# mdolab/adflow

Measured on AMD Instinct MI355X. Metric: Mcells*residual-evals/s, higher is better.
Workload: dtype f64

## Files before the change

adflow_amd/csrc/api.hip:

```cpp
#include <hip/hip_runtime.h>

#include <algorithm>
#include <cmath>
#include <cstdarg>
#include <cstdio>
#include <cstring>
#include <functional>
#include <array>
#include <map>
#include <string>
#include <tuple>
#include <vector>

#include "internal.h"
#include "flow_plan.h"

extern int g_march_kch, g_viscous_tiled, g_inviscid_march, g_roe_march, g_sa_march;
int g_test_fault = 0;
int g_rvec_joint = 1;
int g_pc_fused = 1;
int g_xcd_tiles = 2;

namespace {

// ... 2043 lines not shown
    if (!g_gf_nofit) {
        double tbest = 1.e300;
        const long Tmax = std::max<long>(N, planes / kmin);
        for (long m = 1; m * W <= Tmax + W; ++m) {
            std::vector<int> c;
            split(m * W, c);
            const double t = makespan(c);
            if (t < tbest - 1.e-9) { tbest = t; best = c; }
            if (m > 64) break;
        }
        std::vector<int> one(N, 1);
        if (makespan(one) < tbest) best = one;
    } else {
        best.resize(N);
        const int L = g_march_kch > 0 ? g_march_kch : 32;
        for (int q = 0; q < N; ++q) best[q] = (cols[q].nz + L - 1) / L;
    }
    struct Chunk { int col, k0, k1; };
    std::vector<Chunk> ch;
    for (int q = 0; q < N; ++q) {
        int k = 2;
        for (int e = 0; e < best[q]; ++e) {
            const int len = (cols[q].nz + best[q] - 1 - e) / best[q];
            if (len <= 0) continue;
            ch.push_back(Chunk{q, k, k + len - 1});
            k += len;
        }
    }
    std::stable_sort(ch.begin(), ch.end(), [&](const Chunk& a, const Chunk& b) {
        const int la = a.k1 - a.k0, lb = b.k1 - b.k0;
        if (la != lb) return la > lb;
        if (cols[a.col].slot != cols[b.col].slot) return cols[a.col].slot < cols[b.col].slot;
        if (a.k0 != b.k0) return a.k0 < b.k0;
        return a.col < b.col;
    });
    auto make_table = [&](const std::vector<Chunk>& list, std::pair<int4*, int>* out) -> int {
        const int T = (int)list.size();
        std::vector<int> ord;
        if (round_order(T, W, &ord)) return 1;
        std::vector<int4> phys(ord.size());
        for (size_t p = 0; p < ord.size(); ++p) {
            const int e = ord[p];
            int4 tt;
            if (e >= 0) {
                const Col& c = cols[list[e].col];
                tt.x = c.slot; tt.y = c.bx | (c.by << 16); tt.z = list[e].k0; tt.w = list[e].k1;
            } else { tt.x = -1; tt.y = tt.z = tt.w = 0; }
            phys[p] = tt;
        }
        int n = (int)phys.size();
        while (n > 0 && phys[n - 1].x < 0) --n;
        int4* d = nullptr;
        HIPCHK(hipMalloc((void**)&d, sizeof(int4) * std::max(n, 1)));
        if (n > 0) HIPCHK(hipMemcpy(d, phys.data(), sizeof(int4) * n, hipMemcpyHostToDevice));
        *out = std::make_pair(d, n);
        return 0;
    };
    if (make_table(ch, all)) return 1;
    std::vector<Chunk> in, bd;
    for (const Chunk& c : ch) {
        const Col& q = cols[c.col];
        const int il = q.nx + 1, jl = q.ny + 1, kl = q.nz + 1;
        const int ia = 2 + 60 * q.bx, ib_ = std::min(ia + 59, il), ja = 2 + R * q.by, jb_ = std::min(ja + R - 1, jl);
        const bool interior = (ia - reach >= 2 && ib_ + reach <= il && ja - reach >= 2 && jb_ + reach <= jl && c.k0 - reach >= 2 &&
                               c.k1 + reach <= kl);
        (interior ? in : bd).push_back(c);
    }
    if (make_table(in, in_) || make_table(bd, bd_)) return 1;
    return 0;
}

int ensure_gf_tiles(int level)
{
    if (g_gf_tiles.count(level)) return 0;
    std::pair<int4*, int> a, i, b;
    if (build_chunk_tables(level, 3, 1.5, 1, &a, &i, &b, 2)) return 1;
    g_gf_tiles[level] = a; g_gf_tiles_int[level] = i; g_gf_tiles_bnd[level] = b;
    return 0;
}

int ensure_sa_tiles(int level)
{
    if (g_sa_tiles.count(level)) return 0;
    std::pair<int4*, int> a, i, b;
    if (build_chunk_tables(level, 4, 0.5, 2, &a, &i, &b)) return 1;
    g_sa_tiles[level] = a; g_sa_tiles_int[level] = i; g_sa_tiles_bnd[level] = b;
    return 0;
}

int make_list_host(int level, const int32_t* blk, const int32_t* idx, int ld, int first, int n, std::vector<int>& hb,
                   std::vector<long>& ho)
{
    hb.resize(n);
    ho.resize(n);
    for (int t = 0; t < n; ++t) {
        const int nn = blk[first + t];
        Block* b = find_block(nn, level, 1);
        if (!b) return fail("comm pattern of level %d references unregistered block %d", level, nn);
        const int i = idx[first + t], j = idx[ld + first + t], k = idx[2 * ld + first + t];
        if (i < 0 || i > b->v.ib || j < 0 || j > b->v.jb || k < 0 || k > b->v.kb)
            return fail("comm pattern of level %d: cell (%d,%d,%d) outside block %d", level, i, j, k, nn);
        hb[t] = nn;
        ho[t] = b->v.idx(i, j, k);
    }
    return 0;
}

int upload_list(const std::vector<int>& hb, const std::vector<long>& ho, int** d_blk, long** d_off)
{
    const size_t n = hb.size();
    *d_blk = nullptr;
    *d_off = nullptr;
    if (n == 0) return 0;
    HIPCHK(hipMalloc((void**)d_blk, sizeof(int) * n));
    HIPCHK(hipMalloc((void**)d_off, sizeof(long) * n));
    HIPCHK(hipMemcpy(*d_blk, hb.data(), sizeof(int) * n, hipMemcpyHostToDevice));
    HIPCHK(hipMemcpy(*d_off, ho.data(), sizeof(long) * n, hipMemcpyHostToDevice));
    return 0;
}

int make_list(int level, const int32_t* blk, const int32_t* idx, int ld, int first, int n, int** d_blk, long** d_off)
{
    std::vector<int> hb;
    std::vector<long> ho;
    if (make_list_host(level, blk, idx, ld, first, n, hb, ho)) return 1;
    return upload_list(hb, ho, d_blk, d_off);
}

int build_comm(int level, int nLayers, CommPattern** out)
{
    auto it = g_comm.find(std::make_pair(level, nLayers));
    if (it == g_comm.end()) return fail("no %d-layer comm pattern registered for level %d", nLayers, level);
    CommPattern& cp = it->second;
    *out = &cp;
    if (ensure_table(level)) return 1;
    if (cp.built) return 0;
    const int nc = (int)cp.h_donorBlock.size();
    cp.local.n = nc;
    {
        std::vector<int> db, hb;
        std::vector<long> dof, hof;
        if (make_list_host(level, cp.h_donorBlock.data(), cp.h_donorIdx.data(), nc, 0, nc, db, dof)) return 1;
        if (make_list_host(level, cp.h_haloBlock.data(), cp.h_haloIdx.data(), nc, 0, nc, hb, hof)) return 1;
        std::vector<int> perm(nc);
        for (int t = 0; t < nc; ++t) perm[t] = t;
        std::sort(perm.begin(), perm.end(), [&](int a, int c) { return hb[a] != hb[c] ? hb[a] < hb[c] : hof[a] < hof[c]; });
        std::vector<int> db2(nc), hb2(nc);
        std::vector<long> dof2(nc), hof2(nc);
        for (int t = 0; t < nc; ++t) { db2[t] = db[perm[t]]; dof2[t] = dof[perm[t]]; hb2[t] = hb[perm[t]]; hof2[t] = hof[perm[t]]; }
        if (g_comm_self && nc > 0) {
            cp.local.n = 0;
            CommList s, r;
            s.n = r.n = nc;
            s.peer = r.peer = g_self_rank;
            if (upload_list(db2, dof2, &s.blkA, &s.offA)) return 1;
            if (upload_list(hb2, hof2, &r.blkA, &r.offA)) return 1;
            HIPCHK(hipMalloc((void**)&s.buf, sizeof(double) * 11 * (size_t)nc));
            HIPCHK(hipMalloc((void**)&r.buf, sizeof(double) * 11 * (size_t)nc));
            cp.sends.push_back(s);
            cp.recvs.push_back(r);
        } else {
            if (upload_list(db2, dof2, &cp.local.blkA, &cp.local.offA)) return 1;
            if (upload_list(hb2, hof2, &cp.local.blkB, &cp.local.offB)) return 1;
        }
    }
    const int ns = (int)cp.h_sendProc.size(), nr = (int)cp.h_recvProc.size();
// ... 3167 lines not shown
    if (need_ready()) return 1;
    if (!sums || n < 1 || n > 6) return fail("res_norms: n must be 1..6");
    if (!g_norm_dev) HIPCHK(hipMalloc((void**)&g_norm_dev, sizeof(double) * 8));
    HIPCHK(hipMemsetAsync(g_norm_dev, 0, sizeof(double) * 8, g_stream));
    int rc = for_level(level, [&](Block* b) {
        if (n > b->v.nw) return fail("res_norms: n=%d exceeds nw=%d", n, b->v.nw);
        launch_res_norms(b->v, n, g_norm_dev, g_stream);
        return 0;
    });
    if (rc) return rc;
#ifndef ADFLOW_NO_RCCL
    if (g_nccl && g_nranks > 1) NCCLCHK(ncclAllReduce(g_norm_dev, g_norm_dev, n, ncclDouble, ncclSum, g_nccl, g_stream));
#endif
    HIPCHK(hipMemcpyAsync(sums, g_norm_dev, sizeof(double) * n, hipMemcpyDeviceToHost, g_stream));
    HIPCHK(hipStreamSynchronize(g_stream));
    return 0;
}

int adflow_gpu_event_record(int slot)
{
    if (g_device < 0) return fail("adflow_gpu_init has not been called");
    if (slot < 0 || slot >= 64) return fail("event slot %d out of range", slot);
    HIPCHK(hipEventRecord(g_events[slot], g_stream));
    return 0;
}

int adflow_gpu_event_elapsed_ms(int a, int b, double* ms)
{
    if (a < 0 || a >= 64 || b < 0 || b >= 64 || !ms) return fail("bad event arguments");
    HIPCHK(hipEventSynchronize(g_events[b]));
    float f = 0.f;
    HIPCHK(hipEventElapsedTime(&f, g_events[a], g_events[b]));
    *ms = f;
    return 0;
}

int adflow_gpu_march_stats(int level, double* out, int n)
{
    if (need_ready()) return 1;
    if (!out || n < 4) return fail("march_stats: n = %d (>= 4)", n);
    for (int q = 0; q < n; ++q) out[q] = 0.0;
    if (ensure_gf_tiles(level) || ensure_sa_tiles(level) || ensure_tiles(level)) return 1;
    {
        const auto& tt = g_sa_tiles[level];
        std::vector<int4> h((size_t)tt.second);
        if (tt.second > 0) HIPCHK(hipMemcpy(h.data(), tt.first, sizeof(int4) * h.size(), hipMemcpyDeviceToHost));
        for (const int4& t : h)
            if (t.x >= 0) out[0] += 4.0 * (t.w - t.z + 1);
    }
    {
        const auto& tt = g_gf_tiles[level];
        std::vector<int4> h((size_t)tt.second);
        if (tt.second > 0) HIPCHK(hipMemcpy(h.data(), tt.first, sizeof(int4) * h.size(), hipMemcpyDeviceToHost));
        for (const int4& t : h)
            if (t.x >= 0) out[1] += 4.0 * (t.w - t.z + 3);
    }
    for (auto& kv : g_blocks) {
        if (std::get<0>(kv.first) != level || std::get<1>(kv.first) != 1) continue;
        const BlkView& v = kv.second->v;
        int ntx, nty, ntz;
        euler_march_tiles(v, &ntx, &nty, &ntz);
        out[2] += 4.0 * ntx * nty * (v.nz + ntz);
    }
    return 0;
}

int adflow_gpu_sync(void)
{
    if (g_device < 0) return fail("adflow_gpu_init has not been called");
    HIPCHK(hipGetLastError());
    HIPCHK(hipStreamSynchronize(g_stream));
    return 0;
}

int adflow_gpu_set_tuning(const char* key, int value)
{
    ++g_state_gen;
    if (!key) return fail("null tuning key");
    if (!strcmp(key, "euler_march")) { g_use_march = (value != 0); return 0; }
    if (!strcmp(key, "viscous_tiled")) { g_viscous_tiled = value; return 0; }
    if (!strcmp(key, "inviscid_march")) { g_inviscid_march = value; return 0; }
    if (!strcmp(key, "roe_march")) { g_roe_march = value; return 0; }
    if (!strcmp(key, "sa_march")) { g_sa_march = value; return 0; }
    if (!strcmp(key, "overlap")) { g_overlap = value; return 0; }
    if (!strcmp(key, "max_grid_z")) { g_max_grid_z = (value > 0) ? value : 65535; return 0; }
    if (!strcmp(key, "metric_from_x")) { g_metric_from_x = value; return 0; }
    if (!strcmp(key, "xcd_tiles")) {
        g_xcd_tiles = value;
        if (g_stream) (void)hipStreamSynchronize(g_stream);
        mg_graph_drop();
        for (auto& kv : g_tiles) (void)hipFree(kv.second.first);
        g_tiles.clear();
        return 0;
    }
    if (!strcmp(key, "phase_events")) {
        if (value != 0 && (value < 8 || value > 56)) return fail("phase_events: first slot must be 8..56 (or 0 = off)");
        g_phase_base = value;
        return 0;
    }
    if (!strcmp(key, "march_kch")) {
        if (value < 4) return fail("march_kch must be >= 4");
        g_march_kch = value;
        if (g_stream) (void)hipStreamSynchronize(g_stream);
        mg_graph_drop();
        for (auto* mp : {&g_tiles, &g_gf_tiles, &g_gf_tiles_int, &g_gf_tiles_bnd, &g_sa_tiles, &g_sa_tiles_int, &g_sa_tiles_bnd}) {
            for (auto& kv : *mp) (void)hipFree(kv.second.first);
            mp->clear();
        }
        return 0;
    }
    if (!strcmp(key, "split_eval")) { g_split_eval = value; return 0; }
    if (!strcmp(key, "test_fault")) { g_test_fault = value; g_mgg.failed = false; mg_graph_drop(); return 0; }
    if (!strcmp(key, "ad_cache")) { g_ad_cache = value; if (!value) { if (g_stream) (void)hipStreamSynchronize(g_stream); ad_drop(); } return 0; }
    if (!strcmp(key, "rvec_joint")) { g_rvec_joint = value; return 0; }
    if (!strcmp(key, "jac_snap")) { g_jac_snap = value; return 0; }
    if (!strcmp(key, "pc_fused")) { g_pc_fused = value; mg_graph_drop(); return 0; }
    if (!strcmp(key, "mg_graph")) { g_mg_graph = value; g_mgg.failed = false; mg_graph_drop(); return 0; }
    if (!strcmp(key, "comm_self")) {
        if (g_stream) (void)hipStreamSynchronize(g_stream);
        g_comm_self = value;
        for (auto& kv : g_comm) drop_comm_lists(kv.second);
        return 0;
    }
    if (!strcmp(key, "dadi_pcr")) { g_dadi_pcr = value; mg_graph_drop(); return 0; }
    if (!strcmp(key, "ra_pcr")) { g_ra_pcr = value; mg_graph_drop(); return 0; }
    if (!strcmp(key, "dadi_upd")) { g_dadi_upd = value; mg_graph_drop(); return 0; }
    if (!strcmp(key, "gf_cus")) {
        g_gf_nofit = (value < 0);
        g_num_cus = value > 0 ? value : 0;
        if (g_stream) (void)hipStreamSynchronize(g_stream);
        mg_graph_drop();
        for (auto* mp : {&g_tiles, &g_gf_tiles, &g_gf_tiles_int, &g_gf_tiles_bnd, &g_sa_tiles, &g_sa_tiles_int, &g_sa_tiles_bnd}) {
            for (auto& kv : *mp) (void)hipFree(kv.second.first);
            mp->clear();
        }
        return 0;
    }
    return fail("unknown tuning key '%s'", key);
}

int adflow_gpu_set_async(int on)
{
    g_async = (on != 0);
    return 0;
}

int adflow_gpu_abi_sizes(int* opts_bytes, int* desc_bytes)
{
    if (opts_bytes) *opts_bytes = (int)sizeof(adflow_opts);
    if (desc_bytes) *desc_bytes = (int)sizeof(adflow_block_desc);
    return 0;
}

int adflow_gpu_abi_sizes2(int* bc_subface_bytes, int* comm_pattern_bytes)
{
    if (bc_subface_bytes) *bc_subface_bytes = (int)sizeof(adflow_bc_subface);
    if (comm_pattern_bytes) *comm_pattern_bytes = (int)sizeof(adflow_comm_pattern);
    return 0;
}

}

static void free_side_buffers(void)
{
    free_xsurf();
    if (g_vec_dev) (void)hipFree(g_vec_dev);
    g_vec_dev = nullptr;
    g_vec_elems = 0;
    if (g_norm_dev) (void)hipFree(g_norm_dev);
    g_norm_dev = nullptr;
    if (g_floor_flag_dev) (void)hipFree(g_floor_flag_dev);
    g_floor_flag_dev = nullptr;
    if (g_snapreq.dev) (void)hipFree(g_snapreq.dev);
    g_snapreq = SnapReq();
#ifndef ADFLOW_NO_RCCL
    if (g_nccl) (void)ncclCommDestroy(g_nccl);
    g_nccl = nullptr;
    g_rank = 0;
    g_nranks = 1;
#endif
}
```

adflow_amd/csrc/internal.h:

```cpp
#pragma once
#include <hip/hip_runtime.h>
#include <stdint.h>
#include "../../include/adflow_gpu.h"

#define ADF_PAD0 14

#ifdef HOSTSIM
#define GPTR(T) T*
#else
#define GPTR(T) T __attribute__((address_space(1)))*
#endif

__device__ __forceinline__ double ldg(GPTR(const double) base, unsigned byteoff)
{
    return *(GPTR(const double))((GPTR(const char))base + byteoff);
}
__device__ __forceinline__ void stg(GPTR(double) base, unsigned byteoff, double v)
{
    *(GPTR(double))((GPTR(char))base + byteoff) = v;
}

#ifndef ADF_NR
#define ADF_NR 1
#endif
// ... 311 lines not shown

#include <vector>
struct PcTab {
    long ncell;
    double* fac;
    double* ws;
    const int* nbr;
    const int* vec;
    const int* cblk;
    const int* cbox;
    const JmBlk* blk;
    int* flag;
    int sten[7];
    const double* tsm;
    double turbDiag;
    int asmEnt[23];
    signed char tgt[121];
    double* wsx;
};
int launch_pc_factor(const PcTab& T, int nState, const std::vector<int>& planeStart, hipStream_t s);
enum { PC_MAXW = 4 };
int launch_pc_apply(const PcTab& T, int nState, int transpose, const std::vector<int>& planeStart, const double* r, double* z,
                    hipStream_t s, int nv = 1, long ldr = 0, long ldz = 0);
int launch_pcf_factor(const PcTab& T, int nState, int nEnt, const std::vector<int>& levelStart, hipStream_t s);
int launch_pcf_apply(const PcTab& T, int nState, int nEnt, int transpose, const std::vector<int>& levelStart, const double* r,
                     double* z, hipStream_t s, int nv = 1, long ldr = 0, long ldz = 0);
struct PcMgSten { int s[7]; };
void launch_mg_fine_copy(const JmBlk* src, const JmBlk* dst, int nslots, int maxnx, int maxny, int maxnz, int nState, const PcMgSten& S,
                         const double* tsm, double turbDiag, long N, hipStream_t s);
void launch_mg_coarsen(const JmBlk* fine, const JmBlk* coarse, int nslots, int maxnx, int maxny, int maxnz, int nState, const PcMgSten& S,
                       hipStream_t s);
void launch_mg_restrict(const JmBlk* fine, const JmBlk* coarse, int nslots, int maxnx, int maxny, int maxnz, int nState, const double* r,
                        double* rhs, hipStream_t s);
void launch_mg_residual(const JmBlk* tab, const JmBlk* coarse, int nslots, int maxnx, int maxny, int maxnz, int nState, int transpose,
                        const PcMgSten& S, const double* r, const double* x, double* y, double* res, hipStream_t s);
enum { GM_PARTS = 256 };
int gm_groups(long n);
void launch_gm_mgs(double* w, const double* v, const double* hp, const double* u, double* out, double* hOut, long n, hipStream_t s);
void launch_gm_sum(const double* hp, long n, double* hOut, hipStream_t s);
void launch_gm_axpby(double* y, double a, const double* x, double b, long n, hipStream_t s);
enum { GM_MAXV = 32 };
struct GmCoef { double a[GM_MAXV], b[GM_MAXV]; };
void launch_gm_mgs_multi(double* w, const double* v, const double* hp, const double* u, double* out, double* hOut, long n, long ld,
                         int nvec, hipStream_t s);
void launch_gm_sum_multi(const double* hp, long n, double* hOut, int nvec, hipStream_t s);
void launch_gm_axpby_multi(double* y, long ldy, const double* x, long ldx, const GmCoef& k, long n, int nvec, hipStream_t s);
struct KParams;
enum { ANK_PARTS = 256 };
enum AnkScal {
    ANK_H = 0, ANK_HINV = 1,
    ANK_SUMS = 2,
    ANK_LAMBDA = 5,
    ANK_NORM = 6,
    ANK_NSCAL = 8
};
enum AnkRed {
    ANK_RED_SUMS = 0,
    ANK_RED_MIN = 3 * ANK_PARTS,
    ANK_RED_SCAL = 4 * ANK_PARTS,
    ANK_RED = ANK_RED_SCAL + ANK_NSCAL
};
int ank_groups(long n);
void launch_ank_set_w(const BlkView* tab, int nslots, int maxnx, int maxny, int maxnz, int nS, const double* vec, const double* hv,
                      const double* hdev, const KParams* kp, int* floored, hipStream_t s);
void launch_ank_get_r(const BlkView* tab, int nslots, int maxnx, int maxny, int maxnz, int nS, double* vec, double turbScale, hipStream_t s);
void launch_ank_time_step(const BlkView* tab, int nslots, int maxnx, int maxny, int maxnz, double cfl, double* tsm, long N, hipStream_t s);
void launch_ank_quotient(const BlkView* tab, int nslots, int maxnx, int maxny, int maxnz, int nS, const double* v, const double* r0,
                         const double* tsm, long N, double turbDiag, double turbScale, const double* hdev, double* y, hipStream_t s);
void launch_ank_step(const double* w, const double* v, long n, double errRel, double umin, double* part, double* hdev, hipStream_t s);
void launch_ank_phys(const double* w, double* dw, long ncell, int nS, int flow, int lt, double eps, double tol, double tolTurb,
                     double turbThreshold, double lambda0, double* part, double* out, hipStream_t s);
void launch_ank_set_w_turb(const BlkView* tab, int nslots, int maxnx, int maxny, int maxnz, const double* vec, const double* hv,
                           const double* hdev, const KParams* kp, hipStream_t s);
void launch_ank_get_r_turb(const BlkView* tab, int nslots, int maxnx, int maxny, int maxnz, double* vec, double turbScale, hipStream_t s);
void launch_ank_time_step_turb(const BlkView* tab, int nslots, int maxnx, int maxny, int maxnz, double cfl, double* tsm, hipStream_t s);
void launch_ank_quotient_turb(const BlkView* tab, int nslots, int maxnx, int maxny, int maxnz, const double* v, const double* r0,
                              const double* tsm, double turbDiag, double turbScale, const double* hdev, double* y, hipStream_t s);
long ank_unsteady_groups(int nslots, int maxnx, int maxny, int maxnz);
void launch_ank_unsteady(const BlkView* tab, int nslots, int maxnx, int maxny, int maxnz, int nS, int turb, const double* dW, const double* tsm,
                         long N, double turbDiag, double turbScale, double omega, double* r, double* part, double* out, hipStream_t s);

extern int g_max_grid_z;
extern int g_ra_pcr;
extern int g_dadi_pcr;
inline int level_slots_per_launch(int planes)
{
    const int per = g_max_grid_z / (planes > 0 ? planes : 1);
    return per > 0 ? per : 1;
}
#define LEVEL_SPLIT(nslots, planes, CALL)                                                         \
    {                                                                                             \
        const int per_ = level_slots_per_launch(planes);                                          \
        if ((nslots) > per_) {                                                                    \
            for (int s0_ = 0; s0_ < (nslots); s0_ += per_) {                                      \
                const int n_ = ((nslots) - s0_ < per_) ? (nslots) - s0_ : per_;                   \
                CALL;                                                                             \
            }                                                                                     \
            return;                                                                               \
        }                                                                                         \
    }

void launch_time_step_level(const BlkView* tab, int nslots, int maxnx, int maxny, int maxnz, const KParams& kp, hipStream_t s);
void launch_entropy(const BlkView& b, hipStream_t s);
void launch_inviscid_level(const BlkView* tab, int nslots, int maxnx, int maxny, int maxnz, const KParams& kp, hipStream_t s);
void launch_initres(const BlkView& b, const KParams& kp, int l0, int l1, hipStream_t s);
void launch_viscous(const BlkView& b, const KParams& kp, hipStream_t s);
int viscous_is_tiled();
void launch_sa_march(const BlkView* tab, const int4* tiles, int ntiles, const KParams& kp, hipStream_t s, bool solve);
void launch_visc_march_approx(const BlkView* tab, const int4* tiles, int ntiles, const KParams& kp, hipStream_t s);
bool euler_march_radii_capable(int fwMode, int doScaling, double adis);
void launch_visc_gf(const BlkView* tab, const int4* tiles, int ntiles, const KParams& kp, bool storeGrad, hipStream_t s);
void adf_note_snap(int bits);
int adf_fail(const char* what);
void adf_note_rvec(int bits);
int adf_round_size();
void adf_phase_mark(int i);
void launch_coarse_coordinates_level(const BlkView* ctab, const BlkView* ftab, int nslots, int nx, int ny, int nz, hipStream_t s);
void launch_xhalo_level(const BlkView* tab, int nslots, int nx, int ny, int nz, hipStream_t s);
void launch_xhalo_symm(const BlkView* tab, const BcEntry* ent, const int* order, const BcPhase& ph, hipStream_t s);
void launch_wall_stress(const BlkView* tab, const BcEntry* ent, const int* order, const BcPhase& ph, const KParams& kp, bool formGrad,
                        hipStream_t s);
void launch_viscous_approx(const BlkView& b, const KParams& kp, hipStream_t s);
void launch_face_vectors(const BlkView& b, hipStream_t s);
void launch_sa_residual_level(const BlkView* tab, int nslots, int nx, int ny, int nz, const KParams& kp, hipStream_t s);
void launch_sa_solve_level(const BlkView* tab, int nslots, int nx, int ny, int nz, const KParams& kp, hipStream_t s, bool marchRes = false);
void launch_rk_save_level(const BlkView* tab, int nslots, int maxnx, int maxny, int maxnz, hipStream_t s);
void launch_etot_owned(const BlkView& b, double gammaConstant, hipStream_t s);
void launch_scale_dw_level(const BlkView* tab, int nslots, int maxnx, int maxny, int maxnz, double factor, int timesVol, hipStream_t s);
void launch_source_terms(const BlkView* tab, const int* blk, const long* off, int n, const double Ffact[3], double Qfact, int withBlank,
                         hipStream_t s);
void launch_low_speed_precond_level(const BlkView* tab, int nslots, int maxnx, int maxny, int maxnz, const KParams& kp, hipStream_t s);
void launch_stage_update_level(const BlkView* tab, int nslots, int maxnx, int maxny, int maxnz, const KParams& kp, double scale,
                               int fromWn, hipStream_t s);
void launch_res_averaging_level(const BlkView* tab, int nslots, int maxnx, int maxny, int maxnz, const KParams& kp, hipStream_t s,
                                double scaleDtl = 0.0);
void launch_dadi_level(const BlkView* tab, int nslots, int nx, int ny, int nz, const KParams& kp, hipStream_t s, bool withUpdate = false);
void launch_halo_copy(const BlkView* tab, const int* donorBlk, const long* donorOff, const int* haloBlk, const long* haloOff,
                      int n, unsigned mask, hipStream_t s);
void launch_periodic(const BlkView* tab, const int* blk, const long* off, int n, const double rotMatrix[9], const double rotCenter[3],
                     const double translation[3], int coor, hipStream_t s);
void launch_halo_pack(const BlkView* tab, const int* blk, const long* off, int n, unsigned mask, double* buf, hipStream_t s);
void launch_halo_unpack(const BlkView* tab, const int* blk, const long* off, int n, unsigned mask, const double* buf,
                        hipStream_t s);
int launch_inviscid_march(const BlkView* tab, const int4* tiles, int ntiles, const KParams& kp, hipStream_t s);
int inviscid_march_enabled();
int launch_roe_march(const BlkView* tab, const int4* tiles, int ntiles, const KParams& kp, hipStream_t s);
void launch_pc_march(const BlkView* tab, const int4* tiles, int ntiles, const KParams& kp, int kch, hipStream_t s);
bool roe_march_takes(int limiter);
void launch_euler_march(const BlkView* tab, const int4* tiles, int ntiles, const KParams& kp, hipStream_t s);
void euler_march_tiles(const BlkView& b, int* ntx, int* nty, int* ntz);
void launch_restrict_level(const BlkView* ctab, const BlkView* ftab, int nslots, int nx, int ny, int nz, const KParams& kp, hipStream_t s);
void launch_store_entry_state_level(const BlkView* ctab, int nslots, int nx, int ny, int nz, hipStream_t s);
void launch_forcing_level(const BlkView* ctab, int nslots, int nx, int ny, int nz, double fcoll, hipStream_t s);
void launch_corrections_level(const BlkView* ctab, int nslots, int nx, int ny, int nz, hipStream_t s);
void launch_prolong_update_level(const BlkView* ftab, const BlkView* ctab, int nslots, int nx, int ny, int nz, const KParams& kp,
                                 hipStream_t s);
void launch_set_w(const BlkView& b, const double* vec, double turbFloor, hipStream_t s);
void launch_get_r(const BlkView& b, double* vec, double turbScale, double* sums, hipStream_t s);
void launch_closures(const BlkView& b, const KParams& kp, hipStream_t s);
void launch_closures_level(const BlkView* tab, int nslots, int maxnx, int maxny, int maxnz, const KParams& kp, hipStream_t s,
                           int* floored = nullptr);
void launch_set_w_closures_level(const BlkView* tab, int nslots, int maxnx, int maxny, int maxnz, const double* vec, double turbFloor,
                                 const KParams& kp, int* floored, hipStream_t s);
void launch_set_w_level(const BlkView* tab, int nslots, int maxnx, int maxny, int maxnz, const double* vec, double turbFloor, hipStream_t s);
void launch_get_r_level(const BlkView* tab, int nslots, int maxnx, int maxny, int maxnz, double* vec, double turbScale, double* sums, hipStream_t s);
void launch_entropy_level(const BlkView* tab, int nslots, int maxnx, int maxny, int maxnz, hipStream_t s);
// ... 43 lines not shown
```

adflow_amd/csrc/kernels_sa_march.hip:

```cpp
#ifndef ADF_AD_BUILD
#include "internal.h"
#endif
#include "sa_core.h"

#define GS_BY 4
#ifdef ADF_AD_BUILD
#define GS_MINWG 1
#else
#define GS_MINWG 2
#endif

__device__ __forceinline__ void gs_ld3(GPTR(const adf_real8) a, unsigned o, unsigned nb8, adf_real8 v[3])
{
    v[0] = ldg(a, o); v[1] = ldg(a, o + nb8); v[2] = ldg(a, o + 2 * nb8);
}

#define GS_OUT 60



struct GsCell { double u, v, w, rho, rlv; adf_real8 vol; };
struct GsNbr { double u, v, w, nu, nut; adf_real8 vol; };

struct GsPtrs {
    GPTR(const double) w0; GPTR(const double) w1; GPTR(const double) w2; GPTR(const double) w3; GPTR(const double) w5;
    GPTR(const double) rlv; GPTR(const adf_real8) vol;
    GPTR(const adf_real8) sI; GPTR(const adf_real8) sJ; GPTR(const adf_real8) sK;
    GPTR(const adf_real8) d2wall; GPTR(const adf_real8) volRef;
    unsigned nb8, sj;
};

__device__ __forceinline__ GsCell gs_ld(const GsPtrs& m, unsigned c)
{
    GsCell q;
    q.rho = ldg(m.w0, c); q.u = ldg(m.w1, c); q.v = ldg(m.w2, c); q.w = ldg(m.w3, c);
    q.vol = ldg(m.vol, c); q.rlv = ldg(m.rlv, c);
    return q;
}

__device__ __forceinline__ GsNbr gs_nbr_ld(const GsPtrs& m, unsigned c)
{
    GsNbr q;
    q.u = ldg(m.w1, c); q.v = ldg(m.w2, c); q.w = ldg(m.w3, c);
    q.nu = ldg(m.rlv, c) * rcp_nr(ldg(m.w0, c));
    q.vol = ldg(m.vol, c);
    q.nut = ldg(m.w5, c);
    return q;
}

struct GsNbrRaw { double u, v, w, rlv, rho, nut; adf_real8 vol; };
__device__ __forceinline__ GsNbrRaw gs_nbr_req(const GsPtrs& m, unsigned c)
{
    GsNbrRaw q;
    q.u = ldg(m.w1, c); q.v = ldg(m.w2, c); q.w = ldg(m.w3, c);
    q.rlv = ldg(m.rlv, c); q.rho = ldg(m.w0, c);
    q.vol = ldg(m.vol, c);
    q.nut = ldg(m.w5, c);
    return q;
}
__device__ __forceinline__ GsNbr gs_nbr_of(const GsNbrRaw& r)
{
    GsNbr q;
    q.u = r.u; q.v = r.v; q.w = r.w; q.nu = r.rlv * rcp_nr(r.rho); q.vol = r.vol; q.nut = r.nut;
    return q;
}

__device__ __forceinline__ GsNbr gs_up1(const GsNbr& q)
{
    GsNbr r;
    r.u = lane_up1(q.u); r.v = lane_up1(q.v); r.w = lane_up1(q.w); r.nu = lane_up1(q.nu); r.vol = lane_up1(q.vol); r.nut = lane_up1(q.nut);
    return r;
}
__device__ __forceinline__ GsNbr gs_dn1(const GsNbr& q)
{
    GsNbr r;
    r.u = lane_dn1(q.u); r.v = lane_dn1(q.v); r.w = lane_dn1(q.w); r.nu = lane_dn1(q.nu); r.vol = lane_dn1(q.vol); r.nut = lane_dn1(q.nut);
    return r;
}

template <bool SOLVE, bool RV = false, bool SNAP = false>
__global__ __launch_bounds__(64 * GS_BY, GS_MINWG) void k_sa_march(const BlkView* __restrict__ tab, const int4* __restrict__ tiles, KParams kp)
{
    const int4 tl = tiles[blockIdx.x];
    if (tl.x < 0) return;
    const BlkView& b = tab[tl.x];
    const int lane = threadIdx.x, row = threadIdx.y;
    const int kn0 = tl.z, kn1 = tl.w;
    const int i = (tl.y & 0xffff) * GS_OUT + lane, j = 2 + (tl.y >> 16) * GS_BY + row;
    const int ic = (i < b.ib) ? i : b.ib, jc = (j < b.jb) ? j : b.jb;
    const bool outC = (lane >= 2 && lane <= GS_OUT + 1 && i <= b.il && j <= b.jl);
    const long nb = b.nbox;
    GsPtrs m;
    m.w0 = (GPTR(const double))b.w; m.w1 = m.w0 + nb; m.w2 = m.w1 + nb; m.w3 = m.w2 + nb; m.w5 = m.w3 + 2 * nb;
    m.rlv = (GPTR(const double))b.rlv; m.vol = (GPTR(const adf_real8))b.vol;
    m.sI = (GPTR(const adf_real8))b.sI; m.sJ = (GPTR(const adf_real8))b.sJ; m.sK = (GPTR(const adf_real8))b.sK;
    m.d2wall = (GPTR(const adf_real8))b.d2wall; m.volRef = (GPTR(const adf_real8))b.volRef;
    m.nb8 = 8u * (unsigned)nb; m.sj = 8u * (unsigned)b.ldi;
    GPTR(const adf_real8) xnod = (GPTR(const adf_real8))b.x;
    const adf_real8 mfact = b.mfact;
    const int xn = (kp.metricFromX & 1);
    GPTR(double) dw5 = (GPTR(double))b.dw + 5 * nb;
    GPTR(const uint8_t) flags = (GPTR(const uint8_t))b.flags;
    const unsigned sk = 8u * (unsigned)b.ldk, sj = m.sj;
    const unsigned ojm2 = (jc >= 2) ? 2 * sj : (unsigned)jc * sj, ojp2 = (jc + 2 <= b.jb) ? 2 * sj : (unsigned)(b.jb - jc) * sj;
    const unsigned ojm1 = (jc >= 1) ? sj : 0u, ojp1 = (jc + 1 <= b.jb) ? sj : 0u;
    unsigned c = 8u * (unsigned)(ic + jc * b.ldi + kn0 * b.ldk);
    const bool secondOrd = (kp.orderTurb == 2) && kp.groundLevelIsOne;
    const adf_real8 cb3Inv = 1.0 / kp.sa_cb3;
    adf_real8 sKp[3];
    NgNodes Pn;
    if (xn) {
        ngx_load_x(xnod, c - sk, m.nb8, m.sj, Pn);
        ngx_normal_k(mfact, Pn, sKp);
    } else {
#pragma unroll
        for (int d = 0; d < 3; ++d) sKp[d] = ldg(m.sK, c - sk + d * m.nb8);
    }
    GsCell s0 = gs_ld(m, c);
    GsNbr sm1 = gs_nbr_ld(m, c - sk);
    double n_m2 = ldg(m.w5, c - 2 * sk), n_0 = ldg(m.w5, c), n_p1 = ldg(m.w5, c + sk);
    for (int mm = kn0; mm <= kn1; ++mm) {
        const unsigned ckp2 = (mm + 2 <= b.kb) ? 2 * sk : ((mm + 1 <= b.kb) ? sk : 0u);
        const unsigned ckp1 = (mm + 1 <= b.kb) ? sk : 0u;
        const GsCell sp1 = gs_ld(m, c + ckp1);
        const double n_p2 = ldg(m.w5, c + ckp2);
        const GsNbrRaw rjm = gs_nbr_req(m, c - ojm1), rjp = gs_nbr_req(m, c + ojp1);
        const double n_jm2 = ldg(m.w5, c - ojm2), n_jp2 = ldg(m.w5, c + ojp2);
        const adf_real8 d2w = ldg(m.d2wall, c), volRef0 = ldg(m.volRef, c);
        const int flag0 = flags[c >> 3];
        adf_real8 nI[3], nJm[3], nJ[3], nK[3];
        if (xn) {
            NgNodes Nn;
            ngx_load_x(xnod, c, m.nb8, m.sj, Nn);
            ngx_normals(mfact, Pn, Nn, nI, nJm, nJ, nK);
            Pn = Nn;
        } else {
            gs_ld3(m.sI, c, m.nb8, nI); gs_ld3(m.sJ, c - ojm1, m.nb8, nJm); gs_ld3(m.sJ, c, m.nb8, nJ); gs_ld3(m.sK, c, m.nb8, nK);
        }
        __builtin_amdgcn_sched_barrier(0);
        const adf_real8 sKm[3] = {sKp[0], sKp[1], sKp[2]};
#pragma unroll
        for (int d = 0; d < 3; ++d) sKp[d] = nK[d];
        {
            GsNbr q0;
            q0.u = s0.u; q0.v = s0.v; q0.w = s0.w; q0.nu = s0.rlv * rcp_nr(s0.rho); q0.vol = s0.vol; q0.nut = n_0;
            GsNbr qkp;
            qkp.u = sp1.u; qkp.v = sp1.v; qkp.w = sp1.w; qkp.nu = sp1.rlv * rcp_nr(sp1.rho); qkp.vol = sp1.vol; qkp.nut = n_p1;
            const GsNbr qim = gs_up1(q0), qip = gs_dn1(q0);
            const double n_im2 = lane_up1(qim.nut), n_ip2 = lane_dn1(qip.nut);
            const GsNbr qjm = gs_nbr_of(rjm), qjp = gs_nbr_of(rjp);
            const adf_real8 nIm[3] = {lane_up1(nI[0]), lane_up1(nI[1]), lane_up1(nI[2])};
            double gu[3][3];
            const double qq[3][6] = {{qip.u, qim.u, qjp.u, qjm.u, qkp.u, sm1.u}, {qip.v, qim.v, qjp.v, qjm.v, qkp.v, sm1.v},
                                     {qip.w, qim.w, qjp.w, qjm.w, qkp.w, sm1.w}};
#pragma unroll
            for (int v = 0; v < 3; ++v)
#pragma unroll
                for (int d = 0; d < 3; ++d)
                    gu[v][d] = qq[v][0] * nI[d] - qq[v][1] * nIm[d] + qq[v][2] * nJ[d] - qq[v][3] * nJm[d] + qq[v][4] * nK[d] - qq[v][5] * sKm[d];
            double qjac = 0.0;
            double dvt = sa_source(kp, gu, s0.vol, q0.nu, n_0, d2w, SOLVE ? &qjac : nullptr);
            SaDir dk, dj, di;
#pragma unroll
            for (int d = 0; d < 3; ++d) {
                dk.sm[d] = sKm[d]; dk.sp[d] = nK[d]; dj.sm[d] = nJm[d]; dj.sp[d] = nJ[d]; di.sm[d] = nIm[d]; di.sp[d] = nI[d];
            }
            dk.volm = sm1.vol; dk.volp = qkp.vol; dk.num = sm1.nu; dk.nup = qkp.nu; dk.qsf = 0.0;
            dk.nt[0] = n_m2; dk.nt[1] = sm1.nut; dk.nt[2] = n_0; dk.nt[3] = n_p1; dk.nt[4] = n_p2;
            dj.volm = qjm.vol; dj.volp = qjp.vol; dj.num = qjm.nu; dj.nup = qjp.nu; dj.qsf = 0.0;
            dj.nt[0] = n_jm2; dj.nt[1] = qjm.nut; dj.nt[2] = n_0; dj.nt[3] = qjp.nut; dj.nt[4] = n_jp2;
            di.volm = qim.vol; di.volp = qip.vol; di.num = qim.nu; di.nup = qip.nu; di.qsf = 0.0;
            di.nt[0] = n_im2; di.nt[1] = qim.nut; di.nt[2] = n_0; di.nt[3] = qip.nut; di.nt[4] = n_ip2;
            if (SOLVE) {
                double bmK1 = 0.0, bmK2 = 0.0, bmJ1 = 0.0, bmJ2 = 0.0, bmI1 = 0.0, bmI2 = 0.0;
                if (b.bmt[0] && outC) {
                    if (i == 2) bmI1 = fmax(b.bmt[0][(j - 1) + (long)b.je * (mm - 1)], 0.0);
                    if (i == b.il) bmI2 = fmax(b.bmt[1][(j - 1) + (long)b.je * (mm - 1)], 0.0);
                    if (j == 2) bmJ1 = fmax(b.bmt[2][(i - 1) + (long)b.ie * (mm - 1)], 0.0);
                    if (j == b.jl) bmJ2 = fmax(b.bmt[3][(i - 1) + (long)b.ie * (mm - 1)], 0.0);
                    if (mm == 2) bmK1 = fmax(b.bmt[4][(i - 1) + (long)b.ie * (j - 1)], 0.0);
                    if (mm == b.kl) bmK2 = fmax(b.bmt[5][(i - 1) + (long)b.ie * (j - 1)], 0.0);
                }
                double uuK, uuJ, uuI, c1m, c1p;
                const adf_real8 rbl = flg_blank((uint8_t)flag0);
                GPTR(double) scr = (GPTR(double))b.scratch;
                dvt += sa_advect(dk, s0.vol, s0.u, s0.v, s0.w, secondOrd, &uuK); qjac += fabs(uuK) + ((uuK > 0.0) ? uuK * bmK1 : -uuK * bmK2);
                dvt += sa_advect(dj, s0.vol, s0.u, s0.v, s0.w, secondOrd, &uuJ); qjac += fabs(uuJ) + ((uuJ > 0.0) ? uuJ * bmJ1 : -uuJ * bmJ2);
                dvt += sa_advect(di, s0.vol, s0.u, s0.v, s0.w, secondOrd, &uuI); qjac += fabs(uuI) + ((uuI > 0.0) ? uuI * bmI1 : -uuI * bmI2);
                dvt += sa_diffuse(dk, s0.vol, q0.nu, kp.sa_cb2, cb3Inv, &c1m, &c1p); qjac += c1m + c1p + ((mm == 2) ? c1m * bmK1 : c1p * bmK2);
                if (outC) { stg(scr + 7 * nb, c, (-c1m - fmax(uuK, 0.0)) * rbl); stg(scr + 8 * nb, c, (-c1p + fmin(uuK, 0.0)) * rbl); }
                dvt += sa_diffuse(dj, s0.vol, q0.nu, kp.sa_cb2, cb3Inv, &c1m, &c1p); qjac += c1m + c1p + ((j == 2) ? c1m * bmJ1 : c1p * bmJ2);
                if (outC) { stg(scr + 3 * nb, c, (-c1m - fmax(uuJ, 0.0)) * rbl); stg(scr + 4 * nb, c, (-c1p + fmin(uuJ, 0.0)) * rbl); }
                dvt += sa_diffuse(di, s0.vol, q0.nu, kp.sa_cb2, cb3Inv, &c1m, &c1p); qjac += c1m + c1p + ((i == 2) ? c1m * bmI1 : c1p * bmI2);
                if (outC) { stg(scr + 5 * nb, c, (-c1m - fmax(uuI, 0.0)) * rbl); stg(scr + 6 * nb, c, (-c1p + fmin(uuI, 0.0)) * rbl); }
                if (outC) {
                    stg(scr, c, dvt);
                    stg(scr + nb, c, kp.sa_qqFactor * qjac);
                }
            } else {
                dvt += sa_advect(dk, s0.vol, s0.u, s0.v, s0.w, secondOrd);
                dvt += sa_advect(dj, s0.vol, s0.u, s0.v, s0.w, secondOrd);
                dvt += sa_advect(di, s0.vol, s0.u, s0.v, s0.w, secondOrd);
                dvt += sa_diffuse(dk, s0.vol, q0.nu, kp.sa_cb2, cb3Inv);
                dvt += sa_diffuse(dj, s0.vol, q0.nu, kp.sa_cb2, cb3Inv);
                dvt += sa_diffuse(di, s0.vol, q0.nu, kp.sa_cb2, cb3Inv);
            }
            if (outC) {
                const adf_real8 blank = flg_blank((uint8_t)flag0);
                const double d5 = -volRef0 * dvt * blank;
                if (SNAP) {
                    const SnapSlot ss = kp.snapTab[tl.x];
                    const long m = (long)kp.snapCol * kp.snapN + (5 - kp.snapL0);
                    snap_put((GPTR(adf_real8))ss.snap + m * nb, c, d5 * (1.0 / volRef0) * kp.snapTurbScale);
                } else
                    stg(dw5, c, d5);
#ifndef ADF_AD_BUILD
                if (RV)
                    kp.rvec[b.vecOff + ((((long)(mm - 2) * b.ny + (j - 2)) * b.nx + (i - 2)) * b.nw) + 5] = -dvt * blank * kp.rvecTurbScale;
#endif
            }
        }
        n_m2 = sm1.nut;
        sm1.u = s0.u; sm1.v = s0.v; sm1.w = s0.w; sm1.nu = s0.rlv * rcp_nr(s0.rho); sm1.vol = s0.vol; sm1.nut = n_0;
        s0 = sp1;
        n_0 = n_p1; n_p1 = n_p2;
        c += ckp1;
    }
}


void launch_sa_march(const BlkView* tab, const int4* tiles, int ntiles, const KParams& kp, hipStream_t s, bool solve)
{
    if (ntiles <= 0) return;
    const dim3 grd(ntiles), blk(64, GS_BY, 1);
#ifndef ADF_AD_BUILD
    if (solve) hipLaunchKernelGGL((k_sa_march<true>), grd, blk, 0, s, tab, tiles, kp);
    else if (kp.rvec && !kp.rvecTurbFromDw) {
        hipLaunchKernelGGL((k_sa_march<false, true>), grd, blk, 0, s, tab, tiles, kp);
        adf_note_rvec(2);
    } else
#endif
        if (kp.snapTab) { hipLaunchKernelGGL((k_sa_march<false, false, true>), grd, blk, 0, s, tab, tiles, kp); adf_note_snap(2); }
        else hipLaunchKernelGGL((k_sa_march<false>), grd, blk, 0, s, tab, tiles, kp);
}
```

Before: 4848.

## Stage SA march neighbor loads into LDS via async global-to-LDS DMA

Adds a staged variant of the SA turbulence march kernel that prefetches the next k-plane's stencil data (state, rlv, vol, wall distance, volRef, node coords, flags) straight into LDS with global_load_lds, one 16 KB region per wave. Values are then read from LDS while the following plane's loads are in flight, so global memory latency overlaps with compute. The path is on by default when metrics come from x, and it requires 16-byte-aligned, padded layouts, which are now checked at tile build time. In exchange the kernel uses a large LDS footprint, which can lower occupancy, and it adds more index arithmetic.

```diff
diff --git a/adflow_amd/csrc/api.hip b/adflow_amd/csrc/api.hip
--- a/adflow_amd/csrc/api.hip
+++ b/adflow_amd/csrc/api.hip
@@ -2149,6 +2149,14 @@
 int ensure_sa_tiles(int level)
 {
     if (g_sa_tiles.count(level)) return 0;
+    for (auto& kv : g_blocks) {
+        if (std::get<0>(kv.first) != level || std::get<1>(kv.first) != 1) continue;
+        const BlkView& v = kv.second->v;
+        const uintptr_t bases = (uintptr_t)v.w | (uintptr_t)v.rlv | (uintptr_t)v.vol | (uintptr_t)v.d2wall | (uintptr_t)v.volRef | (uintptr_t)v.x;
+        if ((bases & 15) || ((uintptr_t)v.flags & 3) || (v.ldi & 15) || (v.nbox & 15) || v.nbox < (long)v.ldk * (v.kb + 1) + 16)
+            return fail("block %d of level %d: arrays not laid out for the staged SA march (16-byte bases, ldi and nbox multiples of 16)",
+                        std::get<2>(kv.first), level);
+    }
     std::pair<int4*, int> a, i, b;
     if (build_chunk_tables(level, 4, 0.5, 2, &a, &i, &b)) return 1;
     g_sa_tiles[level] = a; g_sa_tiles_int[level] = i; g_sa_tiles_bnd[level] = b;
@@ -5482,6 +5490,7 @@
     if (!strcmp(key, "inviscid_march")) { g_inviscid_march = value; return 0; }
     if (!strcmp(key, "roe_march")) { g_roe_march = value; return 0; }
     if (!strcmp(key, "sa_march")) { g_sa_march = value; return 0; }
+    if (!strcmp(key, "sa_stage")) { g_sa_stage = value; mg_graph_drop(); return 0; }
     if (!strcmp(key, "overlap")) { g_overlap = value; return 0; }
     if (!strcmp(key, "max_grid_z")) { g_max_grid_z = (value > 0) ? value : 65535; return 0; }
     if (!strcmp(key, "metric_from_x")) { g_metric_from_x = value; return 0; }
@@ -5499,7 +5508,7 @@
         return 0;
     }
     if (!strcmp(key, "march_kch")) {
-        if (value < 4) return fail("march_kch must be >= 4");
+        if (value < 1) return fail("march_kch must be >= 1");
         g_march_kch = value;
         if (g_stream) (void)hipStreamSynchronize(g_stream);
         mg_graph_drop();
diff --git a/adflow_amd/csrc/internal.h b/adflow_amd/csrc/internal.h
--- a/adflow_amd/csrc/internal.h
+++ b/adflow_amd/csrc/internal.h
@@ -417,6 +417,7 @@
 
 extern int g_max_grid_z;
 extern int g_ra_pcr;
+extern int g_sa_stage;
 extern int g_dadi_pcr;
 inline int level_slots_per_launch(int planes)
 {
diff --git a/adflow_amd/csrc/kernels_sa_march.hip b/adflow_amd/csrc/kernels_sa_march.hip
--- a/adflow_amd/csrc/kernels_sa_march.hip
+++ b/adflow_amd/csrc/kernels_sa_march.hip
@@ -2,6 +2,9 @@
 #include "internal.h"
 #endif
 #include "sa_core.h"
+#ifndef ADF_AD_BUILD
+#include "sa_stage.h"
+#endif
 
 #define GS_BY 4
 #ifdef ADF_AD_BUILD
@@ -78,9 +81,36 @@
     return r;
 }
 
-template <bool SOLVE, bool RV = false, bool SNAP = false>
+#ifndef ADF_AD_BUILD
+int g_sa_stage = 1;
+#ifdef HOSTSIM
+#define SS_LDS(T) T*
+#define SS_WAIT_VM0() hostsim::syncthreads()
+#define SS_READS_DONE() hostsim::syncthreads()
+#define SS_DMA(g, l, size) std::memcpy((char*)(l) + (size_t)(hostsim_lane() % 64) * (size), (const void*)(g), (size))
+#else
+#define SS_LDS(T) T __attribute__((address_space(3)))*
+#define SS_WAIT_VM0() asm volatile("s_waitcnt vmcnt(0)" ::: "memory")
+#define SS_READS_DONE() asm volatile("s_waitcnt lgkmcnt(0)" ::: "memory")
+#define SS_DMA(g, l, size) __builtin_amdgcn_global_load_lds((GPTR(const void))(g), (SS_LDS(void))(l), size, 0, 0)
+#endif
+__device__ __forceinline__ void ss_dma16(GPTR(const char) g, SS_LDS(char) l)
+{
+    SS_DMA(g, l, 16);
+}
+__device__ __forceinline__ void ss_dma4(GPTR(const char) g, SS_LDS(char) l)
+{
+    SS_DMA(g, l, 4);
+}
+__device__ __forceinline__ double ss_get(SS_LDS(const char) mine, int slot, int lane) { return *(SS_LDS(const double))(mine + slot * 512 + 8 * lane); }
+#endif
+
+template <bool SOLVE, bool RV = false, bool SNAP = false, bool STAGE = false>
 __global__ __launch_bounds__(64 * GS_BY, GS_MINWG) void k_sa_march(const BlkView* __restrict__ tab, const int4* __restrict__ tiles, KParams kp)
 {
+#ifndef ADF_AD_BUILD
+    __shared__ __attribute__((aligned(16))) char ss_region[STAGE ? GS_BY * SS_WAVE_BYTES : 16];
+#endif
     const int4 tl = tiles[blockIdx.x];
     if (tl.x < 0) return;
     const BlkView& b = tab[tl.x];
@@ -98,7 +128,7 @@
     m.nb8 = 8u * (unsigned)nb; m.sj = 8u * (unsigned)b.ldi;
     GPTR(const adf_real8) xnod = (GPTR(const adf_real8))b.x;
     const adf_real8 mfact = b.mfact;
-    const int xn = (kp.metricFromX & 1);
+    const int xn = STAGE ? 1 : (kp.metricFromX & 1);
     GPTR(double) dw5 = (GPTR(double))b.dw + 5 * nb;
     GPTR(const uint8_t) flags = (GPTR(const uint8_t))b.flags;
     const unsigned sk = 8u * (unsigned)b.ldk, sj = m.sj;
@@ -107,6 +137,31 @@
     unsigned c = 8u * (unsigned)(ic + jc * b.ldi + kn0 * b.ldk);
     const bool secondOrd = (kp.orderTurb == 2) && kp.groundLevelIsOne;
     const adf_real8 cb3Inv = 1.0 / kp.sa_cb3;
+#ifndef ADF_AD_BUILD
+    const SsBox sbox = {b.ib, b.jb, b.kb, b.ldi, (long)b.ldk, nb};
+    const int wrow = wave_uniform(row), jcu = wave_uniform(jc);
+    SS_LDS(char) mine = (SS_LDS(char))ss_region + (STAGE ? wrow * SS_WAVE_BYTES : 0);
+    const unsigned sspc = STAGE ? 8u * (unsigned)ss_pair_col(sbox, tl.y & 0xffff, lane) : 0u;
+    const unsigned ssfo = STAGE ? (unsigned)(jcu * b.ldi + ss_flag_col(sbox, tl.y & 0xffff, lane)) : 0u;
+    GPTR(const char) ssb[SS_NARR8];
+    ssb[SS_W] = (GPTR(const char))m.w0; ssb[SS_RLV] = (GPTR(const char))m.rlv; ssb[SS_VOL] = (GPTR(const char))m.vol;
+    ssb[SS_D2W] = (GPTR(const char))m.d2wall; ssb[SS_VOLREF] = (GPTR(const char))m.volRef; ssb[SS_X] = (GPTR(const char))xnod;
+    auto ss_request = [&](int mq) {
+#pragma unroll
+        for (int q = 0; q < SS_NFULL; ++q) {
+            const unsigned sa = ss_row_off(sbox, jcu, 2 * q) + ss_plane_off(sbox, mq, 2 * q);
+            const unsigned sb = ss_row_off(sbox, jcu, 2 * q + 1) + ss_plane_off(sbox, mq, 2 * q + 1);
+            ss_dma16(ssb[ss_pieces[2 * q].arr] + (((lane < 32) ? sa : sb) + sspc), mine + q * 1024);
+        }
+        if (lane < 32) {
+#pragma unroll
+            for (int p = 2 * SS_NFULL; p < SS_NPIECE; ++p)
+                ss_dma16(ssb[ss_pieces[p].arr] + (ss_row_off(sbox, jcu, p) + ss_plane_off(sbox, mq, p) + sspc), mine + p * 512);
+        }
+        if (lane < 16) ss_dma4((GPTR(const char))flags + (ssfo + (unsigned)mq * (unsigned)b.ldk), mine + SS_FLAG_SLOT * 512);
+    };
+    if (STAGE) ss_request(kn0);
+#endif
     adf_real8 sKp[3];
     NgNodes Pn;
     if (xn) {
@@ -122,13 +177,43 @@
     for (int mm = kn0; mm <= kn1; ++mm) {
         const unsigned ckp2 = (mm + 2 <= b.kb) ? 2 * sk : ((mm + 1 <= b.kb) ? sk : 0u);
         const unsigned ckp1 = (mm + 1 <= b.kb) ? sk : 0u;
-        const GsCell sp1 = gs_ld(m, c + ckp1);
-        const double n_p2 = ldg(m.w5, c + ckp2);
-        const GsNbrRaw rjm = gs_nbr_req(m, c - ojm1), rjp = gs_nbr_req(m, c + ojp1);
-        const double n_jm2 = ldg(m.w5, c - ojm2), n_jp2 = ldg(m.w5, c + ojp2);
-        const adf_real8 d2w = ldg(m.d2wall, c), volRef0 = ldg(m.volRef, c);
-        const int flag0 = flags[c >> 3];
+        GsCell sp1;
+        double n_p2, n_jm2, n_jp2;
+        GsNbrRaw rjm, rjp;
+        adf_real8 d2w, volRef0;
+        int flag0;
         adf_real8 nI[3], nJm[3], nJ[3], nK[3];
+#ifndef ADF_AD_BUILD
+        if (STAGE) {
+            SS_WAIT_VM0();
+            sp1.rho = ss_get(mine, SSV_RHO_P1, lane); sp1.u = ss_get(mine, SSV_U_P1, lane); sp1.v = ss_get(mine, SSV_V_P1, lane);
+            sp1.w = ss_get(mine, SSV_W_P1, lane); sp1.vol = ss_get(mine, SSV_VOL_P1, lane); sp1.rlv = ss_get(mine, SSV_RLV_P1, lane);
+            n_p2 = ss_get(mine, SSV_NT_P2, lane); n_jm2 = ss_get(mine, SSV_NT_JM2, lane); n_jp2 = ss_get(mine, SSV_NT_JP2, lane);
+            rjm.u = ss_get(mine, SSV_U_JM1, lane); rjm.v = ss_get(mine, SSV_V_JM1, lane); rjm.w = ss_get(mine, SSV_W_JM1, lane);
+            rjm.rlv = ss_get(mine, SSV_RLV_JM1, lane); rjm.rho = ss_get(mine, SSV_RHO_JM1, lane); rjm.vol = ss_get(mine, SSV_VOL_JM1, lane);
+            rjm.nut = ss_get(mine, SSV_NT_JM1, lane);
+            rjp.u = ss_get(mine, SSV_U_JP1, lane); rjp.v = ss_get(mine, SSV_V_JP1, lane); rjp.w = ss_get(mine, SSV_W_JP1, lane);
+            rjp.rlv = ss_get(mine, SSV_RLV_JP1, lane); rjp.rho = ss_get(mine, SSV_RHO_JP1, lane); rjp.vol = ss_get(mine, SSV_VOL_JP1, lane);
+            rjp.nut = ss_get(mine, SSV_NT_JP1, lane);
+            d2w = ss_get(mine, SSV_D2W, lane); volRef0 = ss_get(mine, SSV_VOLREF, lane);
+            flag0 = *(SS_LDS(const uint8_t))(mine + SS_FLAG_SLOT * 512 + lane);
+            NgNodes Nn;
+            Nn.a[0] = ss_get(mine, SSV_XA0, lane); Nn.a[1] = ss_get(mine, SSV_XA1, lane); Nn.a[2] = ss_get(mine, SSV_XA2, lane);
+            Nn.b[0] = ss_get(mine, SSV_XB0, lane); Nn.b[1] = ss_get(mine, SSV_XB1, lane); Nn.b[2] = ss_get(mine, SSV_XB2, lane);
+            SS_READS_DONE();
+            if (mm < kn1) ss_request(mm + 1);
+            __builtin_amdgcn_sched_barrier(0);
+            ngx_normals(mfact, Pn, Nn, nI, nJm, nJ, nK);
+            Pn = Nn;
+        } else
+#endif
+        {
+        sp1 = gs_ld(m, c + ckp1);
+        n_p2 = ldg(m.w5, c + ckp2);
+        rjm = gs_nbr_req(m, c - ojm1); rjp = gs_nbr_req(m, c + ojp1);
+        n_jm2 = ldg(m.w5, c - ojm2); n_jp2 = ldg(m.w5, c + ojp2);
+        d2w = ldg(m.d2wall, c); volRef0 = ldg(m.volRef, c);
+        flag0 = flags[c >> 3];
         if (xn) {
             NgNodes Nn;
             ngx_load_x(xnod, c, m.nb8, m.sj, Nn);
@@ -138,6 +223,7 @@
             gs_ld3(m.sI, c, m.nb8, nI); gs_ld3(m.sJ, c - ojm1, m.nb8, nJm); gs_ld3(m.sJ, c, m.nb8, nJ); gs_ld3(m.sK, c, m.nb8, nK);
         }
         __builtin_amdgcn_sched_barrier(0);
+        }
         const adf_real8 sKm[3] = {sKp[0], sKp[1], sKp[2]};
 #pragma unroll
         for (int d = 0; d < 3; ++d) sKp[d] = nK[d];
@@ -229,17 +315,38 @@
 }
 
 
+#ifndef ADF_AD_BUILD
+template <bool STAGE>
+struct SaLaunch {
+    template <bool SOLVE, bool RV = false, bool SNAP = false>
+    static constexpr auto k_sa_march = &::k_sa_march<SOLVE, RV, SNAP, STAGE>;
+    static void go(const BlkView* tab, const int4* tiles, const KParams& kp, hipStream_t s, dim3 grd, dim3 blk)
+    {
+        if (kp.rvec && !kp.rvecTurbFromDw) {
+            hipLaunchKernelGGL((k_sa_march<false, true>), grd, blk, 0, s, tab, tiles, kp);
+            adf_note_rvec(2);
+        } else if (kp.snapTab) {
+            hipLaunchKernelGGL((k_sa_march<false, false, true>), grd, blk, 0, s, tab, tiles, kp);
+            adf_note_snap(2);
+        } else
+            hipLaunchKernelGGL((k_sa_march<false>), grd, blk, 0, s, tab, tiles, kp);
+    }
+};
+#endif
+
 void launch_sa_march(const BlkView* tab, const int4* tiles, int ntiles, const KParams& kp, hipStream_t s, bool solve)
 {
-    if (ntiles <= 0) return;
+    if (ntiles <= 0) {
+        if (kp.snapTab) adf_note_snap(2);
+        return;
+    }
     const dim3 grd(ntiles), blk(64, GS_BY, 1);
 #ifndef ADF_AD_BUILD
     if (solve) hipLaunchKernelGGL((k_sa_march<true>), grd, blk, 0, s, tab, tiles, kp);
-    else if (kp.rvec && !kp.rvecTurbFromDw) {
-        hipLaunchKernelGGL((k_sa_march<false, true>), grd, blk, 0, s, tab, tiles, kp);
-        adf_note_rvec(2);
-    } else
-#endif
-        if (kp.snapTab) { hipLaunchKernelGGL((k_sa_march<false, false, true>), grd, blk, 0, s, tab, tiles, kp); adf_note_snap(2); }
-        else hipLaunchKernelGGL((k_sa_march<false>), grd, blk, 0, s, tab, tiles, kp);
-}
+    else if (g_sa_stage != 0 && (kp.metricFromX & 1)) SaLaunch<true>::go(tab, tiles, kp, s, grd, blk);
+    else SaLaunch<false>::go(tab, tiles, kp, s, grd, blk);
+#else
+    if (kp.snapTab) { hipLaunchKernelGGL((k_sa_march<false, false, true>), grd, blk, 0, s, tab, tiles, kp); adf_note_snap(2); }
+    else hipLaunchKernelGGL((k_sa_march<false>), grd, blk, 0, s, tab, tiles, kp);
+#endif
+}
diff --git a/adflow_amd/csrc/sa_stage.h b/adflow_amd/csrc/sa_stage.h
--- /dev/null
+++ b/adflow_amd/csrc/sa_stage.h
@@ -0,0 +1,71 @@
+#pragma once
+
+#if defined(__HIPCC__) || defined(HOSTSIM)
+#define SS_HD __host__ __device__
+#else
+#define SS_HD
+#endif
+
+enum { SS_W, SS_RLV, SS_VOL, SS_D2W, SS_VOLREF, SS_X, SS_NARR8, SS_FLAGS = SS_NARR8 };
+struct SsPiece { int arr, comp, dj, dk; };
+enum { SS_NFULL = 13, SS_NHALF = 5, SS_NPIECE = 2 * SS_NFULL + SS_NHALF, SS_FLAG_SLOT = SS_NPIECE, SS_WAVE_BYTES = 16384 };
+enum {
+    SSV_RHO_P1, SSV_U_P1, SSV_V_P1, SSV_W_P1,
+    SSV_NT_P2, SSV_NT_JM2, SSV_NT_JP2, SSV_NT_JM1,
+    SSV_U_JM1, SSV_V_JM1, SSV_W_JM1, SSV_RHO_JM1,
+    SSV_U_JP1, SSV_V_JP1, SSV_W_JP1, SSV_RHO_JP1,
+    SSV_RLV_P1, SSV_RLV_JM1, SSV_VOL_P1, SSV_VOL_JM1,
+    SSV_XA0, SSV_XA1, SSV_XA2, SSV_XB0, SSV_XB1, SSV_XB2,
+    SSV_NT_JP1, SSV_RLV_JP1, SSV_VOL_JP1, SSV_D2W, SSV_VOLREF
+};
+static constexpr SsPiece ss_pieces[SS_NPIECE] = {
+    {SS_W, 0, 0, 1}, {SS_W, 1, 0, 1}, {SS_W, 2, 0, 1}, {SS_W, 3, 0, 1},
+    {SS_W, 5, 0, 2}, {SS_W, 5, -2, 0}, {SS_W, 5, 2, 0}, {SS_W, 5, -1, 0},
+    {SS_W, 1, -1, 0}, {SS_W, 2, -1, 0}, {SS_W, 3, -1, 0}, {SS_W, 0, -1, 0},
+    {SS_W, 1, 1, 0}, {SS_W, 2, 1, 0}, {SS_W, 3, 1, 0}, {SS_W, 0, 1, 0},
+    {SS_RLV, 0, 0, 1}, {SS_RLV, 0, -1, 0}, {SS_VOL, 0, 0, 1}, {SS_VOL, 0, -1, 0},
+    {SS_X, 0, 0, 0}, {SS_X, 1, 0, 0}, {SS_X, 2, 0, 0}, {SS_X, 0, -1, 0}, {SS_X, 1, -1, 0}, {SS_X, 2, -1, 0},
+    {SS_W, 5, 1, 0}, {SS_RLV, 0, 1, 0}, {SS_VOL, 0, 1, 0}, {SS_D2W, 0, 0, 0}, {SS_VOLREF, 0, 0, 0}};
+
+struct SsBox { int ib, jb, kb, ldi; long ldk, nbox; };
+
+SS_HD inline int ss_row(const SsBox& g, int jc, int dj)
+{
+    if (dj == -2) return jc >= 2 ? jc - 2 : 0;
+    if (dj == -1) return jc >= 1 ? jc - 1 : jc;
+    if (dj == 1) return jc + 1 <= g.jb ? jc + 1 : jc;
+    if (dj == 2) return jc + 2 <= g.jb ? jc + 2 : g.jb;
+    return jc;
+}
+SS_HD inline int ss_plane(const SsBox& g, int mm, int dk)
+{
+    if (dk == 1) return mm + 1 <= g.kb ? mm + 1 : mm;
+    if (dk == 2) return mm + 2 <= g.kb ? mm + 2 : (mm + 1 <= g.kb ? mm + 1 : mm);
+    return mm;
+}
+SS_HD inline int ss_pair_col(const SsBox& g, int bx, int lane)
+{
+    const int c = 60 * bx + 2 * (lane & 31), last = g.ib & ~1;
+    return c < last ? c : last;
+}
+SS_HD inline int ss_flag_col(const SsBox& g, int bx, int lane)
+{
+    const int c = 60 * bx + 4 * (lane & 15), last = g.ib & ~3;
+    return c < last ? c : last;
+}
+SS_HD inline unsigned ss_row_off(const SsBox& g, int jc, int p)
+{
+    const SsPiece pc = ss_pieces[p];
+    return 8u * (unsigned)((long)pc.comp * g.nbox + (long)ss_row(g, jc, pc.dj) * g.ldi);
+}
+SS_HD inline unsigned ss_lane_off(const SsBox& g, int bx, int jc, int lane, int p) { return ss_row_off(g, jc, p) + 8u * (unsigned)ss_pair_col(g, bx, lane); }
+SS_HD inline unsigned ss_plane_off(const SsBox& g, int mm, int p) { return 8u * (unsigned)((long)ss_plane(g, mm, ss_pieces[p].dk) * g.ldk); }
+SS_HD inline unsigned ss_flag_off(const SsBox& g, int bx, int jc, int lane, int mm)
+{
+    return (unsigned)((long)mm * g.ldk + (long)jc * g.ldi + ss_flag_col(g, bx, lane));
+}
+SS_HD inline int ss_piece_of(int q, int lane)
+{
+    if (q < SS_NFULL) return 2 * q + (lane >> 5);
+    return lane < 32 ? 2 * SS_NFULL + (q - SS_NFULL) : -1;
+}
```

Result: no change. 4856, median of 4 (+0.2%).
